# xiejihong0306/collision-detect-GJK-EPA

Hardware: AMD Instinct MI355X
Metric: M convex-pair GJK+EPA queries/sec at 1/2/4/8 MI355X; % HBM roofline (higher is better)
Workload: dtype f64

## Files before the change

### collision-detect-gjk-epa_amd/csrc/gjkepa_kernel.h

```cpp
#pragma once
#include <hip/hip_runtime.h>

#include <cstddef>
#include <cstdint>

#ifndef GJKEPA_G0_G
#define GJKEPA_G0_G 4
#endif
#ifndef GJKEPA_G0_K
#define GJKEPA_G0_K 8
#endif
#ifndef GJKEPA_G0_MINW
#define GJKEPA_G0_MINW 2
#endif
#ifndef GJKEPA_G1_G
#define GJKEPA_G1_G 16
#endif
#ifndef GJKEPA_G1_K
#define GJKEPA_G1_K 8
#endif
#ifndef GJKEPA_G1_MINW
#define GJKEPA_G1_MINW 3
#endif
#ifndef GJKEPA_G2_G
// ... 100 lines not shown
#endif
#ifndef GJKEPA_E5_FCAP
#define GJKEPA_E5_FCAP 416
#endif
#ifndef GJKEPA_E5_MINW
#define GJKEPA_E5_MINW 1
#endif
#ifndef GJKEPA_Q_VCAP
#define GJKEPA_Q_VCAP 40
#endif
#ifndef GJKEPA_Q_FCAP
#define GJKEPA_Q_FCAP 64
#endif
#ifndef GJKEPA_C0_G
#define GJKEPA_C0_G 8
#endif
#ifndef GJKEPA_C0_K
#define GJKEPA_C0_K 4
#endif
#ifndef GJKEPA_C0_MINW
#define GJKEPA_C0_MINW 3
#endif
#ifndef GJKEPA_C1_G
#define GJKEPA_C1_G 64
#endif
#ifndef GJKEPA_C1_K
#define GJKEPA_C1_K 4
#endif
#ifndef GJKEPA_C1_MINW
#define GJKEPA_C1_MINW 3
#endif
#ifndef GJKEPA_EPA_SEED
#define GJKEPA_EPA_SEED 1
#endif
#ifndef GJKEPA_GJK_META
#define GJKEPA_GJK_META 1
#endif
#ifndef GJKEPA_CONTACT_META
#define GJKEPA_CONTACT_META 1
#endif
#ifndef GJKEPA_E1_PRIO
#define GJKEPA_E1_PRIO 2
#endif
#ifndef GJKEPA_HORIZON_W16
#define GJKEPA_HORIZON_W16 1
#endif
#ifndef GJKEPA_SCREEN_SINGLE
#define GJKEPA_SCREEN_SINGLE 1
#endif
#ifndef GJKEPA_EPA_HPACK
#define GJKEPA_EPA_HPACK 1
#endif
#ifndef GJKEPA_PAD_V0
#define GJKEPA_PAD_V0 1
#endif
#ifndef GJKEPA_EMPTY_INF
#define GJKEPA_EMPTY_INF 1
#endif
#ifndef GJKEPA_DOTS_FMAX
#define GJKEPA_DOTS_FMAX 1
#endif
#ifndef GJKEPA_EPA_PLACE
#define GJKEPA_EPA_PLACE 1
#endif
#ifndef GJKEPA_LDS_SKEW
#define GJKEPA_LDS_SKEW 1
// ... 25 lines not shown
#ifndef GJKEPA_E2_LH
#define GJKEPA_E2_LH 0
#endif
#ifndef GJKEPA_E3_LH
#define GJKEPA_E3_LH 1
#endif
#ifndef GJKEPA_E4_LH
#define GJKEPA_E4_LH 1
#endif
#ifndef GJKEPA_E5_LH
#define GJKEPA_E5_LH 0
#endif
#ifndef GJKEPA_C0_LH
#define GJKEPA_C0_LH 1
#endif
#ifndef GJKEPA_C1_LH
#define GJKEPA_C1_LH 1
#endif
#ifndef GJKEPA_CONTACT_OVERLAP
#define GJKEPA_CONTACT_OVERLAP 1
#endif
#define GJKEPA_GJK_TIERS 3
#define GJKEPA_EPA_TIERS 6
#define GJKEPA_CONTACT_TIERS 2

#define GJKEPA_WS_COUNTERS 40
#define GJKEPA_WS_TALLY 48
#define GJKEPA_ROUTE_DONE 0
#define GJKEPA_ROUTE_GJK1 1
#define GJKEPA_ROUTE_EPA0 0x10
#define GJKEPA_ROUTE_CT0 0x20
#define GJKEPA_ROUTE_CT(t) (GJKEPA_ROUTE_CT0 + 2 * (t))
#define GJKEPA_ROUTE_REDO 0x2E

#ifndef GJKEPA_PARK
#define GJKEPA_PARK 1
#endif
#define GJKEPA_PARK_VC 72
#define GJKEPA_PARK_FC 128
#define GJKEPA_PARK_HDR 128
#define GJKEPA_PARK_BYTES (GJKEPA_PARK_HDR + 3 * 8 * GJKEPA_PARK_VC + 2 * 4 * GJKEPA_PARK_FC)

#define GJKEPA_GRID_UNITS (-2)

struct gjkepa_gjk_args {
    const void* verts;
    const int64_t* hull_off;
    const int32_t* hull_cnt;
    const int32_t* pairs;
    int64_t n_pairs;
    uint8_t* route;
    int route_code;
    uint32_t* ctr;
    int claim;
    uint32_t* tally;
    uint32_t* warm;
    void* out;
    int grid;
    int num_cus;
    uint32_t guard;
};

struct gjkepa_epa_args {
    int version;
    double tol_ff;
    const void* verts;
// ... 85 lines not shown
```

### collision-detect-gjk-epa_amd/csrc/gjkepa_kernel.hip

```cpp
#include <hip/hip_runtime.h>

#include <cfloat>
#include <cmath>
#include <cstdint>
#include <type_traits>

#include "../../include/gjkepa.h"
#include "gjkepa_kernel.h"
#include "gk_common.h"

#ifdef GK_PART
#define GK_IN(p) (GK_PART == (p))
#else
#define GK_IN(p) 1
#endif

namespace gk {

constexpr int ST_DEFER = 100;
constexpr int ST_REDO = 103;
constexpr int ST_PARKED = 104;

DEV void gk_lds_fence() { asm volatile("" ::: "memory"); }
#ifndef GJKEPA_SCREEN_FENCE_MIN_G
#define GJKEPA_SCREEN_FENCE_MIN_G 32
#endif
#ifndef GJKEPA_DOTS_FENCE_MIN_G
#define GJKEPA_DOTS_FENCE_MIN_G 64
#endif

template <typename T> DEV constexpr bool certify() { return sizeof(T) == 4; }
template <typename T> DEV bool redo_status(int r, bool last_tier) {
    if constexpr (!certify<T>()) return false;
    return r == ST_REDO || r == GJKEPA_STATUS_EPA_MAXITER || r == GJKEPA_STATUS_DEGENERATE || (r == ST_DEFER && last_tier);
}

[[maybe_unused]] static __constant__ double kDirTab[100][3] = {
#include "dirtab.inc"
};

#ifdef GJKEPA_DIAG_STAMPS
constexpr int kStamps = 32;
__device__ unsigned long long g_stamps[kStamps];
__shared__ unsigned long long s_stamp[kStamps + 1];
DEV void stamp(int id) {
    const uint64_t t = __builtin_amdgcn_s_memtime();
    const uint64_t act = __ballot(1);
    if ((uint64_t)lane_id() == (uint64_t)__builtin_ctzll(act)) { s_stamp[id] += t - s_stamp[kStamps]; s_stamp[kStamps] = t; }
}
DEV void stamp_begin() {
    if (lane_id() == 0) {
        for (int i = 0; i < kStamps; ++i) s_stamp[i] = 0;
        s_stamp[kStamps] = __builtin_amdgcn_s_memtime();
    }
}
DEV void stamp_end() {
    if (lane_id() == 0)
        for (int i = 0; i < kStamps; ++i) if (s_stamp[i]) atomicAdd(&g_stamps[i], s_stamp[i]);
}
#define GK_STAMP(id) stamp(id)
#define GK_STAMP_BEGIN() stamp_begin()
#define GK_STAMP_END() stamp_end()
#elif defined(GJKEPA_DIAG_MARKERS)
#define GK_STAMP(id) asm volatile("; GKMARK %0" ::"n"(id))
#define GK_STAMP_BEGIN() ((void)0)
#define GK_STAMP_END() ((void)0)
#else
// ... 693 lines not shown
        if (f < FC && !(F.fv[r] & kEmpty)) {
            int rk = 0;
            for (int j = 0; j < hw; ++j) rk += E.x.o.key[j] < F.key[r];
            E.x.o.ord[rk] = F.fv[r];
        }
    }
    __builtin_amdgcn_wave_barrier();
    T sx = 0, sy = 0, sz = 0;
    for (int j = 0; j < 3; ++j)
        for (int f = 0; f < nf; ++f) {
            const V3<T> q = c.vert((int)((E.x.o.ord[f] >> (8 * j)) & 0xffu));
            sx += q.x; sy += q.y; sz += q.z;
        }
    __builtin_amdgcn_wave_barrier();
    const T cnt = (T)(nf * 3);
    return vmk<T>(sx / cnt, sy / cnt, sz / cnt);
}

constexpr int ST_CONT = 101;

template <typename T, int R> struct EpaState {
    Faces<T, R> F;
    int nv, hw, nf, F1, iters;
    uint32_t kbase;
    T minv;
    V3<T> dir;
    bool neg;
    int av;
    bool unchanged;
    T hsup;
};
#define EPAST_T EpaState<T, (FC + G - 1) / G>

CTX_T DEV int epa_begin(CTX& c, EPAST_T& S, V3<T> s0, V3<T> s1, V3<T> s2, V3<T> s3) {
    constexpr int R = (FC + G - 1) / G;
    auto& E = c.L.u.e;
    const V3<T> O = zero3<T>();
    const int gl = c.g.gl;
#pragma unroll
    for (int r = 0; r < R; ++r) {
        free_slot(S.F, r);
        const int f = r * G + gl;
        if (f < FC) E.dsv[f] = qnan<T>();
    }
    S.nv = 0; S.hw = 0; S.nf = 0; S.kbase = 0; S.iters = 1; S.F1 = 4; S.unchanged = false;
    const int fq = gl & 3;
    const V3<T> fa = fq == 3 ? s1 : s0, fb = (fq == 0 || fq == 2) ? s1 : s2, fc = fq == 0 ? s2 : s3;
    const V3<T> nq = uninml(fa, fb, fc);
    if (c.g.unib(quad_any(is_zero_nml(nq)))) return GJKEPA_STATUS_DEGENERATE;
    const T dq = fabs(dot(vsub(O, fa), nq));
    const T d0 = qbcast<0>(dq), d1 = qbcast<1>(dq), d2 = qbcast<2>(dq), d3 = qbcast<3>(dq);
    T minv = d0;
    int kmin = 0;
    if (d1 < minv) { minv = d1; kmin = 1; }
    if (d2 < minv) { minv = d2; kmin = 2; }
    if (d3 < minv) { minv = d3; kmin = 3; }
    V3<T> dir = quad_pick(fq == kmin, nq);
    const V3<T> a1 = kmin == 3 ? s1 : s0;
    if (gl < 4) E.dsv[gl] = dq;
    T dt = dot(vsub(a1, O), dir);
    if (c.g.unib(fabs(dt) < Tol<T>::ZO)) {
        const T sx = ((((((((((s0.x + s0.x) + s0.x) + s1.x) + s1.x) + s2.x) + s1.x) + s2.x) + s2.x) + s3.x) + s3.x) + s3.x;
        const T sy = ((((((((((s0.y + s0.y) + s0.y) + s1.y) + s1.y) + s2.y) + s1.y) + s2.y) + s2.y) + s3.y) + s3.y) + s3.y;
        const T sz = ((((((((((s0.z + s0.z) + s0.z) + s1.z) + s1.z) + s2.z) + s1.z) + s2.z) + s2.z) + s3.z) + s3.z) + s3.z;
        const T cnt = (T)12;
        dt = dot(vsub(a1, vmk<T>(sx / cnt, sy / cnt, sz / cnt)), dir);
    }
    if (c.g.unib(dt <= -Tol<T>::ZO)) dir = vneg(dir);
    GK_STAMP(SE_IT1);
    const V3<T> sp = support(c, dir);
    if constexpr (certify<T>()) { S.minv = minv; S.hsup = dot(sp, dir); }
    const bool two = c.g.unib(fabs(minv) < Tol<T>::ZO);
    const bool u1 = !veq(s1, s0);
    const bool u2 = !veq(s2, s0) && !veq(s2, s1);
    const bool u3 = !veq(s3, s0) && !veq(s3, s1) && !veq(s3, s2);
    const int i1 = 1, i2 = u1 ? 2 : 1, i3 = i2 + (u2 ? 1 : 0), isp = i3 + (u3 ? 1 : 0);
    int m = isp + 1;
    V3<T> sq = zero3<T>();
    if (two) { sq = support(c, vneg(dir)); ++m; }
    V3<T> q = s0;
    bool w = gl == 0;
    if (u1 && gl == i1) { q = s1; w = true; }
    if (u2 && gl == i2) { q = s2; w = true; }
    if (u3 && gl == i3) { q = s3; w = true; }
    if (gl == isp) { q = sp; w = true; }
    if (two && gl == isp + 1) { q = sq; w = true; }
    if (w) { E.vx[gl] = q.x; E.vy[gl] = q.y; E.vz[gl] = q.z; }
    __builtin_amdgcn_wave_barrier();
    GK_STAMP(SE_IT1);
    return hull_build(c, S.F, S.kbase, S.hw, S.nv, S.nf, m);
}

constexpr int ST_FALLBACK = 102;
CTX_T DEV int epa_seed(CTX& c, EPAST_T& S, V3<T> s0, V3<T> s1, V3<T> s2, V3<T> s3) {
    constexpr int R = (FC + G - 1) / G;
    auto& E = c.L.u.e;
    const V3<T> O = zero3<T>();
    const int gl = c.g.gl;
    const bool distinct = !veq(s1, s0) && !veq(s2, s0) && !veq(s2, s1) && !veq(s3, s0) && !veq(s3, s1) && !veq(s3, s2);
    if (!c.g.unib(distinct)) return ST_FALLBACK;
    const V3<T> e1 = vsub(s1, s0);
    const T l1 = norm2(e1);
    if (!c.g.unib(l1 > Tol<T>::HULL)) return ST_FALLBACK;
    const V3<T> c2 = cross(e1, vsub(s2, s0));
    if (!c.g.unib(norm2(c2) / l1 > Tol<T>::HULL)) return ST_FALLBACK;
    const V3<T> pn = utzvec(c2);
    if (!c.g.unib(fabs(dot(vsub(s3, s0), pn)) > Tol<T>::HULL)) return ST_FALLBACK;
#pragma unroll
    for (int r = 0; r < R; ++r) {
        free_slot(S.F, r);
        const int f = r * G + gl;
        if (f < FC) E.dsv[f] = qnan<T>();
    }
    S.iters = 1; S.F1 = 4; S.unchanged = false;
    const int fq = gl & 3;
    const V3<T> fa = fq == 3 ? s1 : s0, fb = (fq == 0 || fq == 2) ? s1 : s2, fc = fq == 0 ? s2 : s3;
    const V3<T> nq = uninml(fa, fb, fc);
    if (c.g.unib(quad_any(is_zero_nml(nq)))) return GJKEPA_STATUS_DEGENERATE;
    const T dq = fabs(dot(vsub(O, fa), nq));
    const T d0 = qbcast<0>(dq), d1 = qbcast<1>(dq), d2 = qbcast<2>(dq), d3 = qbcast<3>(dq);
    T minv = d0;
    int kmin = 0;
    if (d1 < minv) { minv = d1; kmin = 1; }
    if (d2 < minv) { minv = d2; kmin = 2; }
    if (d3 < minv) { minv = d3; kmin = 3; }
    V3<T> dir = quad_pick(fq == kmin, nq);
    const V3<T> a1 = kmin == 3 ? s1 : s0;
    if (gl < 4) E.dsv[gl] = dq;
    T dt = dot(vsub(a1, O), dir);
    if (c.g.unib(fabs(dt) < Tol<T>::ZO)) {
        const T sx = ((((((((((s0.x + s0.x) + s0.x) + s1.x) + s1.x) + s2.x) + s1.x) + s2.x) + s2.x) + s3.x) + s3.x) + s3.x;
        const T sy = ((((((((((s0.y + s0.y) + s0.y) + s1.y) + s1.y) + s2.y) + s1.y) + s2.y) + s2.y) + s3.y) + s3.y) + s3.y;
        const T sz = ((((((((((s0.z + s0.z) + s0.z) + s1.z) + s1.z) + s2.z) + s1.z) + s2.z) + s2.z) + s3.z) + s3.z) + s3.z;
        const T cnt = (T)12;
        dt = dot(vsub(a1, vmk<T>(sx / cnt, sy / cnt, sz / cnt)), dir);
    }
    if (c.g.unib(dt <= -Tol<T>::ZO)) dir = vneg(dir);
    S.dir = dir;
    S.minv = minv;
    if (gl < 4) {
        const V3<T> q = gl == 0 ? s0 : gl == 1 ? s1 : gl == 2 ? s2 : s3;
        E.vx[gl] = q.x; E.vy[gl] = q.y; E.vz[gl] = q.z;
    }
    const V3<T> cen = centroid4(s0, s1, s2, s3);
    bool bad = false;
    if (gl < 4) {
        int a = gl == 3 ? 1 : 0, b = (gl == 0 || gl == 2) ? 1 : 2, d = gl == 0 ? 2 : 3;
        const V3<T> Pa = vsel(gl == 3, s1, s0);
        V3<T> Pb = vsel(gl == 0 || gl == 2, s1, s2);
        V3<T> Pd = vsel(gl == 0, s2, s3);
        const V3<T> n0 = cross(vsub(Pb, Pa), vsub(Pd, Pb));
        if (dot(n0, vsub(Pa, cen)) < T(0)) { int t = b; b = d; d = t; const V3<T> q = Pb; Pb = Pd; Pd = q; }
        const V3<T> n = uninml(Pa, Pb, Pd);
        bad = is_zero_nml(n);
        S.F.nx[0] = n.x; S.F.ny[0] = n.y; S.F.nz[0] = n.z;
        S.F.d[0] = dot(vsub(zero3<T>(), Pa), n);
        S.F.fv[0] = (uint32_t)a | ((uint32_t)b << 8) | ((uint32_t)d << 16);
        S.F.key[0] = (uint32_t)gl;
    }
    __builtin_amdgcn_wave_barrier();
    if (c.g.any(bad)) return GJKEPA_STATUS_DEGENERATE;
    S.nv = 4; S.nf = 4; S.kbase = 4; S.hw = 4;
    GK_STAMP(SE_IT1);
    return 0;
}

CTX_T DEV int epa_close(CTX& c, EPAST_T& S, T& depth, V3<T>& normal) {
    const int F2 = S.nf;
    const T prev = S.minv;
    face_argmin(c, S.F, S.minv, S.dir, S.neg, S.av);
    if constexpr (certify<T>()) {
        if (c.g.unib(S.minv < prev - Tol<T>::CERT_DROP * prev)) return ST_REDO;
    }
    V3<T> dir2 = S.dir;
    if (c.g.unib(!S.neg && S.minv > T(0))) dir2 = vneg(dir2);
    bool stop;
    if (S.F1 == F2) stop = S.unchanged || sorted_equal(c, S.F, S.hw);
    else stop = S.F1 > F2;
    GK_STAMP(SE_TERM);
    if constexpr (certify<T>()) {
        if (stop) {
            constexpr int R = (FC + G - 1) / G;
            bool out = false;
#pragma unroll
            for (int r = 0; r < R; ++r) out = out || (!(S.F.fv[r] & kEmpty) && !(S.F.d[r] < T(0)));
            const float sc = c.vmax_a + c.vmax_b;
            const uint32_t bw = c.L.u.e.bestv;
// ... 107 lines not shown
    const T* vx = reinterpret_cast<const T*>(rec + GJKEPA_PARK_HDR);
    const uint32_t* fv = reinterpret_cast<const uint32_t*>(rec + kParkFaces);
    S.nv = c.g.uni((int)hdr[0]); S.hw = c.g.uni((int)hdr[1]); S.nf = c.g.uni((int)hdr[2]); S.F1 = c.g.uni((int)hdr[3]);
    S.iters = c.g.uni((int)hdr[4]); S.kbase = hdr[5]; S.neg = hdr[6] != 0; S.av = (int)hdr[7]; gjk_it = hdr[8];
    S.dir = vmk<T>(tv[0], tv[1], tv[2]);
    S.minv = tv[3];
    S.hsup = tv[4];
    S.unchanged = false;
    for (int i = gl; i < S.nv; i += G) {
        E.vx[i] = vx[i];
        E.vy[i] = vx[GJKEPA_PARK_VC + i];
        E.vz[i] = vx[2 * GJKEPA_PARK_VC + i];
    }
    __builtin_amdgcn_wave_barrier();
#pragma unroll
    for (int r = 0; r < R; ++r) {
        const int f = r * G + gl;
        free_slot(S.F, r);
        if (f < S.hw) {
            const uint32_t w = fv[f];
            if (!(w & kEmpty)) {
                const V3<T> U = c.vert((int)(w & 0xffu)), W = c.vert((int)((w >> 8) & 0xffu)), P = c.vert((int)((w >> 16) & 0xffu));
                const V3<T> n = uninml(U, W, P);
                S.F.nx[r] = n.x; S.F.ny[r] = n.y; S.F.nz[r] = n.z;
                S.F.d[r] = dot(vsub(zero3<T>(), U), n);
                S.F.fv[r] = w;
                S.F.key[r] = fv[GJKEPA_PARK_FC + f];
            }
        }
    }
}

CTX_T DEV int epa(CTX& c, V3<T> s0, V3<T> s1, V3<T> s2, V3<T> s3, T& depth, V3<T>& normal, int& iters, int& nf,
                  bool park = false, ParkCtl pk = {}, const unsigned char* rec = nullptr, uint32_t* gjk_it = nullptr) {
    EPAST_T S;
    int st;
    if (rec) {
        epa_resume(c, S, rec, *gjk_it);
        st = epa_grow(c, S, false);
    } else {
        st = epa_begin(c, S, s0, s1, s2, s3);
        if (st == 0) st = ST_CONT;
    }
    while (st == ST_CONT) {
        st = epa_close(c, S, depth, normal);
        if (st != ST_CONT) break;
        if constexpr (VC <= GJKEPA_PARK_VC && FC <= GJKEPA_PARK_FC) {
            if (park && park_now(c, S, pk)) { st = ST_PARKED; break; }
        }
        st = epa_grow(c, S, false);
    }
    iters = S.iters;
    nf = S.nf;
    return st;
}

CTX_T DEV void scan_top2(CTX& c, int side, V3<T> n, int& i0, int& i1) {
    T mx = -Tol<T>::BIG;
    i0 = -1; i1 = -1;
    const int cnt = side ? c.nb : c.na;
    for (int i = 0; i < cnt; ++i) {
        T t = dot(n, side ? c.B(i) : c.A(i));
        if (t > mx - Tol<T>::PT) { mx = t; i1 = i0; i0 = i; }
    }
    if (i1 == -1) i1 = i0;
}

CTX_T DEV T hull_dot_max(CTX& c, int side, V3<T> n) {
    T mx = -Tol<T>::BIG;
#pragma unroll
    for (int k = 0; k < K; ++k) {
        int i = k * G + c.g.gl;
        const V3<T> p = side ? c.BV(k) : c.AV(k);
        T t = n.x * p.x + n.y * p.y + n.z * p.z;
// ... 440 lines not shown
    k1 = (k == 0 || k == 3) ? c2 : c1;
    k2 = k == 2 ? c2 : c3;
    k3 = km;
}

constexpr double kWarmMargin = 1e-6;
constexpr uint32_t kWarmMiss = 0xFFFFFFFEu;
CTX_T DEV bool warm_start(CTX& c, const uint32_t* w, uint32_t* kc) {
    uint32_t code[4];
    bool ok = true;
#pragma unroll
    for (int i = 0; i < 4; ++i) {
        code[i] = w[i];
        ok = ok && code[i] != kStale && (int)(code[i] & 0xffffu) < c.na && (int)(code[i] >> 16) < c.nb;
    }
    if (!c.g.unib(ok)) return false;
    const V3<T> s0 = decode_pt(c, code[0]), s1 = decode_pt(c, code[1]), s2 = decode_pt(c, code[2]), s3 = decode_pt(c, code[3]);
    const V3<T> M = centroid4(s0, s1, s2, s3), O = zero3<T>();
    const V3<T> P[4] = {s0, s1, s2, s3};
    const int F[4][3] = {{0, 2, 3}, {0, 1, 3}, {0, 1, 2}, {1, 2, 3}};
    bool inside = true;
#pragma unroll
    for (int f = 0; f < 4; ++f) {
        V3<T> n = face_nml(P[F[f][0]], P[F[f][1]], P[F[f][2]]);
        if (dot(n, vsub(P[F[f][0]], M)) < T(0)) n = vneg(n);
        inside = inside && dot(vsub(P[F[f][0]], O), n) > T(kWarmMargin);
    }
    if (!c.g.unib(inside)) return false;
#pragma unroll
    for (int i = 0; i < 4; ++i) kc[i] = code[i];
    return true;
}

CTX_T DEV int gjk_phase(CTX& c, uint32_t* kc, int& gjk_it, bool try_axis = false) {
    const V3<T> O = zero3<T>();
    auto& L = c.L;
    const int gl = c.g.gl;
    gjk_it = 0;
    bool axis_sep = false;
    {
        T cs[(6 + G - 1) / G];
#pragma unroll
        for (int j0 = 0; j0 < 6; j0 += G) {
            const int j = j0 + gl;
            cs[j0 / G] = T(0);
            if (j < 6) {
                const int h = j / 3, ax = j - 3 * (j / 3);
#if GJKEPA_HULL_AOS
                const TH* col = &L.hv[h][0].x + ax;
                constexpr int CS = 4;
#else
                const TH* col = ax == 0 ? L.hx[h] : ax == 1 ? L.hy[h] : L.hz[h];
                constexpr int CS = 1;
#endif
                const int n = h ? c.nb : c.na;
                T sum = 0;
                int i = 0;
                for (; i + 8 <= n; i += 8) {
                    TH v[8];
#pragma unroll
                    for (int u = 0; u < 8; ++u) v[u] = col[CS * (i + u)];
#pragma unroll
                    for (int u = 0; u < 8; ++u) sum += (T)v[u];
                }
                for (; i < n; ++i) sum += (T)col[CS * i];
                cs[j0 / G] = sum / (T)n;
            }
// ... 22 lines not shown
#pragma unroll
            for (int k = 0; k < K; ++k) {
                const int i = k * G + gl;
                const V3<T> pa = c.AV(k), pb = c.BV(k);
                const T ta = d.x * pa.x + d.y * pa.y + d.z * pa.z;
                const T tb = d.x * pb.x + d.y * pb.y + d.z * pb.z;
                if (i < c.na && ta > amax) amax = ta;
                if (i < c.nb && tb < bmin) bmin = tb;
            }
            amax = gmax<G>(amax);
            bmin = gmin<G>(bmin);
            const T margin = sizeof(T) == 8 ? T(kWarmMargin) : T(1e-4);
            axis_sep = c.g.unib(bmin - amax > margin * norm2(d));
        }
    }
    V3<T> s0 = O, s1 = O, s2 = O, s3 = O;
    uint32_t k0 = kStale, k1 = kStale, k2 = kStale, k3 = kStale;
    V3<T> dir;
    for (int iter = 1;; ++iter) {
        if (iter > 99) return PH_MISS;
        dir = vmk<T>((T)kDirTab[iter - 1][0], (T)kDirTab[iter - 1][1], (T)kDirTab[iter - 1][2]);
        s0 = support_pt(c, dir, k0);
        dir = vneg(dir);
        s1 = support_pt(c, dir, k1);
        if (!c.g.unib(allclose8(s0, s1))) break;
    }
    dir = vec_pl(O, s0, s1);
    s2 = support_pt(c, dir, k2);
    if (c.g.unib(allclose8(s2, s0) || allclose8(s2, s1))) return PH_MISS;
    dir = utzvec(cross(vsub(s1, s0), vsub(s2, s1)));
    const T vd = dot(vsub(O, s2), dir);
    bool enter = false;
    if (c.g.unib(fabs(vd) < Tol<T>::PT) && c.g.unib(inside_tri(s0, s1, s2, O))) enter = true;
    const int q = gl & 3;
    V3<T> nq = zero3<T>();
    T mdq = 0;
    if (!enter) {
        if (c.g.unib(vd < T(0))) dir = vneg(dir);
        s3 = support_pt(c, dir, k3);
        const V3<T> n = uninml(s0, s1, s2);
        if (c.g.unib(is_zero_nml(n))) return GJKEPA_STATUS_DEGENERATE;
        if (c.g.unib(fabs(dot(vsub(s3, s0), n)) < Tol<T>::PT)) return PH_MISS;
        nq = quad_normal(q, s0, s1, s2, s3, mdq);
        if (c.g.unib(quad_inside(q, s0, s1, s2, s3, nq))) enter = true;
    }
    GK_STAMP(SG_INIT);
    if (!enter && axis_sep) return PH_MISS;
    if (!enter) {
        constexpr int HS = (12 + G - 1) / G;
        T h1[HS], h2[HS];
#pragma unroll
        for (int t = 0; t < HS; ++t) { h1[t] = 0; h2[t] = 0; }
        const uint64_t lowg = G == 64 ? ~0ull : ((1ull << (G & 63)) - 1ull);
        const int sh = c.g.lane & ~(G - 1);
        for (int it = 1;; ++it) {
            gjk_it = it;
            if (it > 50) return PH_MISS;
#pragma unroll
            for (int t = 0; t < HS; ++t) {
                const int j = t * G + gl;
                h2[t] = h1[t];
                h1[t] = simplex_coord(j < 12 ? j : 0, s0, s1, s2, s3);
            }
            GK_STAMP(SG_CHK);
            update_simplex_c(c, nq, s0, s1, s2, s3, k0, k1, k2, k3);
            nq = quad_normal(q, s0, s1, s2, s3, mdq);
            GK_STAMP(SG_UPD);
            if (c.g.unib(qbcast<2>(mdq) < Tol<T>::PT)) return PH_MISS;
            const V3<T> n = vmk<T>(qbcast<2>(nq.x), qbcast<2>(nq.y), qbcast<2>(nq.z));
            if (c.g.unib(fabs(dot(vsub(s3, s0), n)) < Tol<T>::PT)) return PH_MISS;
            if (c.g.unib(quad_inside(q, s0, s1, s2, s3, nq))) break;
            uint32_t e1 = 0, e2 = 0;
#pragma unroll
            for (int t = 0; t < HS; ++t) {
                const int j = t * G + gl;
                const T cur = simplex_coord(j < 12 ? j : 0, s0, s1, s2, s3);
                e1 |= (uint32_t)((__ballot(fabs(cur - h1[t]) < Tol<T>::PT) >> sh) & lowg) << (t * G);
                e2 |= (uint32_t)((__ballot(fabs(cur - h2[t]) < Tol<T>::PT) >> sh) & lowg) << (t * G);
            }
            e1 &= 0xFFFu;
            e2 &= 0xFFFu;
            bool over = true;
#pragma unroll
            for (int p = 0; p < 4; ++p) over = over && (((e1 >> (3 * p)) & 7u) == 7u || ((e2 >> (3 * p)) & 7u) == 7u);
            if (c.g.unib(over)) return PH_MISS;
        }
        GK_STAMP(SG_CHK);
    }
    kc[0] = k0; kc[1] = k1; kc[2] = k2; kc[3] = k3;
    return PH_HIT;
}

CTX_T DEV int epa_phase(CTX& c, const uint32_t* kc, T& depth, V3<T>& n, uint32_t& diag_epa, bool park = false,
                        ParkCtl pk = {}, const unsigned char* rec = nullptr, uint32_t* gjk_it = nullptr) {
    V3<T> s0 = zero3<T>(), s1 = s0, s2 = s0, s3 = s0;
    if (!rec) { s0 = decode_pt(c, kc[0]); s1 = decode_pt(c, kc[1]); s2 = decode_pt(c, kc[2]); s3 = decode_pt(c, kc[3]); }
    depth = 0;
    n = zero3<T>();
    int eit = 0, nf = 0;
    const int st = epa(c, s0, s1, s2, s3, depth, n, eit, nf, park, pk, rec, gjk_it);
    diag_epa = ((uint32_t)(eit & 0xff) << 8) | ((uint32_t)(nf & 0xffff) << 16);
    return st;
}

CTX_T DEV int contact_phase(CTX& c, T depth, V3<T> n, int version, T tol_ff, T* o13) {
    int st;
    int ia, ib;
    GK_STAMP(SE_TERM);
    DotSet<T, K> D;
    support_dots(c, n, D, ia, ib);
    GK_STAMP(SE_NEAR);
    V3<T> pt = zero3<T>();
    int type = (version == 1 || version == 2) ? collision_type(c, D, tol_ff) : 0;
    if (version == 1) st = contact_v1(c, n, D, pt);
    else if (version == 2) st = contact_v2(c, D, pt);
    else if (version == 3) { V3<T> nw; st = contact_v3(c, n, pt, nw); n = nw; }
    else st = GJKEPA_STATUS_BAD_VERSION;
    GK_STAMP(SE_CONT);
    if (st) return st;
    if (version == 3) type = collision_type(c, n, tol_ff);
    GK_STAMP(SE_TYPE);
    const V3<T> q1 = c.A(ia), q2 = c.B(ib);
    __builtin_amdgcn_wave_barrier();
    o13[0] = depth;
    o13[1] = n.x; o13[2] = n.y; o13[3] = n.z;
    o13[4] = pt.x; o13[5] = pt.y; o13[6] = pt.z;
    o13[7] = q1.x; o13[8] = q1.y; o13[9] = q1.z;
    o13[10] = q2.x; o13[11] = q2.y; o13[12] = q2.z;
    return -type;
}

CTX_T DEV bool load_hulls(CTX& c, const TH* __restrict__ pa, const TH* __restrict__ pb) {
    const int gl = c.g.gl;
// ... 233 lines not shown
    GK_STAMP_BEGIN();
    if (tier_empty(a.tally, a.route_code)) return;
    tally_begin();
    const int claim = pick_claim(a.tally, a.route_code, a.n_pairs, a.claim);
    auto body = [&](int64_t pair, const PairMeta& pm) {
        GK_STAMP(SG_ROUTE);
        Ctx<T, TIn, G, K, 0, 0, LH> c{L, grp};
        const int na = grp.uni(pm.na), nb = grp.uni(pm.nb);
        T o13[13];
#pragma unroll
        for (int i = 0; i < 13; ++i) o13[i] = T(0);
        uint8_t next = 0;
        if (na < 1 || nb < 1 || na > GJKEPA_MAX_HULL_VERTS || nb > GJKEPA_MAX_HULL_VERTS) {
            store_record<G, T>(a.out, pair, gl, o13, 0, 0, GJKEPA_STATUS_BAD_INPUT, 0u);
            if (WARM && gl < 4) a.warm[4 * pair + gl] = kStale;
        } else if (na > K * G || nb > K * G) {
            next = (uint8_t)((na > nb ? na : nb) <= GJKEPA_G1_G * GJKEPA_G1_K ? GJKEPA_ROUTE_GJK1 : GJKEPA_ROUTE_GJK1 + 1);
        } else {
            c.na = na;
            c.nb = nb;
            const bool bad_in = load_hulls(c, verts + pm.oa, verts + pm.ob);
            GK_STAMP(SG_LOAD);
            if (bad_in) {
                store_record<G, T>(a.out, pair, gl, o13, 0, 0, GJKEPA_STATUS_BAD_INPUT, 0u);
                if (WARM && gl < 4) a.warm[4 * pair + gl] = kStale;
            } else {
                uint32_t kc[4];
                int gjk_it = 0;
                int r = PH_MISS;
                bool warm_hit = false;
                if constexpr (WARM) {
                    if (a.warm[4 * pair] != kWarmMiss) warm_hit = warm_start(c, a.warm + 4 * pair, kc);
                }
                if (warm_hit) r = PH_HIT;
                else r = gjk_phase(c, kc, gjk_it, GJKEPA_AXIS_REJECT != 0);
                __builtin_amdgcn_wave_barrier();
                GK_STAMP(SG_CHK);
                if (WARM && gl < 4)
                    a.warm[4 * pair + gl] = r == PH_HIT ? (gl == 0 ? kc[0] : gl == 1 ? kc[1] : gl == 2 ? kc[2] : kc[3])
                                          : (r == PH_MISS && gl == 0) ? kWarmMiss : kStale;
                if (r == PH_HIT) {
#pragma unroll
                    for (int j0 = 0; j0 < 6; j0 += G) {
                        const int j = j0 + gl;
                        const uint32_t word = j == 0 ? kc[0] : j == 1 ? kc[1] : j == 2 ? kc[2] : j == 3 ? kc[3] : j == 4 ? (uint32_t)gjk_it : 0u;
                        if (j < 6) reinterpret_cast<uint32_t*>(a.out)[pair * (sizeof(T) == 8 ? 32 : 16) + j] = word;
                    }
                    next = (uint8_t)(GJKEPA_ROUTE_EPA0 + epa_tier_for(na > nb ? na : nb));
                } else if (r == PH_MISS) {
                    store_record<G, T>(a.out, pair, gl, o13, 0, 0, 0, 0u);
                } else if (certify<T>()) {
                    next = GJKEPA_ROUTE_REDO;
                } else {
                    store_record<G, T>(a.out, pair, gl, o13, 1, 0, r, (uint32_t)(gjk_it & 0xff));
                }
            }
        }
        if (gl == 0) { a.route[pair] = next; tally_route(next); }
        __builtin_amdgcn_wave_barrier();
        GK_STAMP(SG_STORE);
    };
#if GJKEPA_GJK_META
    for_each_routed_pair<G, true>(grp, a.n_pairs, a.route, a.route_code, a.ctr, claim, false, body, a.pairs, a.hull_cnt,
                                  a.hull_off);
#else
    for_each_routed_pair<G>(grp, a.n_pairs, a.route, a.route_code, a.ctr, claim, false, [&](int64_t pair) {
        const int32_t ha = a.pairs[2 * pair], hb = a.pairs[2 * pair + 1];
        body(pair, PairMeta{a.hull_cnt[ha], a.hull_cnt[hb], a.hull_off[ha], a.hull_off[hb]});
    });
#endif
    GK_STAMP(SG_ROUTE);
    tally_end(a.tally);
    GK_STAMP_END();
}

DEV int contact_tier_for(int nmax) { return nmax <= GJKEPA_C0_G * GJKEPA_C0_K ? 0 : 1; }

template <typename TIn, typename T, int G, int K, int VC, int FC, int MINW, bool LH, int PR>
__global__ __launch_bounds__(64, MINW) void epa_kernel(const gjkepa_epa_args a) {
// ... 1 lines not shown
    extern __shared__ __align__(16) unsigned char smem[];
    const Grp<G> grp;
    L_t& L = *reinterpret_cast<L_t*>(smem + lds_stride<L_t, G>() * (grp.lane / G));
    const int gl = grp.gl;
    const TIn* verts = (const TIn*)a.verts;
    GK_GUARD(2, a.route_code);
    GK_STAMP_BEGIN();
    if (tier_empty(a.tally, a.route_code)) return;
    tally_begin();
    const int claim = pick_claim(a.tally, a.route_code, a.n_pairs, a.claim);
    for_each_routed_pair<G>(grp, a.n_pairs, a.route, a.route_code, a.ctr, claim, false, [&](int64_t pair) {
        GK_STAMP(SE_ROUTE);
        Ctx<T, TIn, G, K, VC, FC, LH> c{L, grp};
        const int32_t ha = a.pairs[2 * pair], hb = a.pairs[2 * pair + 1];
        c.na = grp.uni(a.hull_cnt[ha]);
        c.nb = grp.uni(a.hull_cnt[hb]);
        uint32_t* slot = reinterpret_cast<uint32_t*>(a.out) + pair * (sizeof(T) == 8 ? 32 : 16);
        uint32_t kc[4];
        kc[0] = slot[0]; kc[1] = slot[1]; kc[2] = slot[2]; kc[3] = slot[3];
        const uint32_t gjk_it = slot[4];
        load_hulls(c, verts + a.hull_off[ha], verts + a.hull_off[hb]);
        T depth;
        V3<T> n;
        uint32_t de = 0;
        GK_STAMP(SE_LOAD);
#ifdef GJKEPA_DIAG_GJK_ONLY
        const int r = GJKEPA_STATUS_DEGENERATE;
        depth = 0; n = zero3<T>();
#else
        const uint32_t parked = (PR & 2) && a.park ? slot[5] : 0u;
        uint32_t it_park = gjk_it;
        const ParkCtl pk{a.park, a.park_ctr, a.park_cap, gjk_it, slot};
        const bool can_park = (PR & 1) && a.park && a.next_code >= 0;
        const int r = (c.na > G * K || c.nb > G * K) ? ST_DEFER
                    : epa_phase(c, kc, depth, n, de, can_park, pk,
                                parked ? a.park + (size_t)(parked - 1) * GJKEPA_PARK_BYTES : nullptr, &it_park);
#endif
        __builtin_amdgcn_wave_barrier();
        const uint32_t diag = (gjk_it & 0xffu) | de;
        uint8_t next = 0;
        if ((r == ST_DEFER || r == ST_PARKED) && a.next_code >= 0) {
            next = (uint8_t)(GJKEPA_ROUTE_EPA0 + epa_tier_for(c.na > c.nb ? c.na : c.nb, a.next_code - GJKEPA_ROUTE_EPA0, VC));
        } else if (redo_status<T>(r, a.next_code < 0)) {
            next = GJKEPA_ROUTE_REDO;
        } else if (r == 0) {
            T* rec = reinterpret_cast<T*>(slot);
            if (gl < 4) rec[gl] = gl == 0 ? depth : gl == 1 ? n.x : gl == 2 ? n.y : n.z;
            if (gl == 4) slot[sizeof(T) == 8 ? 27 : 14] = diag;
            next = (uint8_t)(a.ct_base + contact_tier_for(c.na > c.nb ? c.na : c.nb));
        } else {
            T o13[13];
#pragma unroll
            for (int i = 0; i < 13; ++i) o13[i] = T(0);
            store_record<G, T>(a.out, pair, gl, o13, 1, 0, r == ST_DEFER ? GJKEPA_STATUS_DEGENERATE : r, diag);
        }
        if (gl == 0) { a.route[pair] = next; tally_route(next); }
        __builtin_amdgcn_wave_barrier();
        GK_STAMP(SE_STORE);
    });
    GK_STAMP(SE_ROUTE);
    tally_end(a.tally);
    GK_STAMP_END();
}

struct PairQueue {
    const uint8_t* route;
    Units U;
    int64_t ch, p0;
    uint32_t* ctr;
// ... 70 lines not shown
            if (gl == 4 % G) slot[sizeof(T) == 8 ? 27 : 14] = diag;
            next = (uint8_t)(a.ct_base + contact_tier_for(c.na > c.nb ? c.na : c.nb));
        } else {
            T o13[13];
#pragma unroll
            for (int i = 0; i < 13; ++i) o13[i] = T(0);
            store_record<G, T>(a.out, pair, gl, o13, 1, 0, r == ST_DEFER ? GJKEPA_STATUS_DEGENERATE : r, diag);
        }
        if (gl == 0) { a.route[pair] = next; tally_route(next); }
    };
    for (;;) {
        const uint64_t idle = __ballot(gl == 0 && !active);
        const int nidle = popc(idle);
        bool fresh = false;
        if (!q.done && (nidle >= REFILL || nidle == NG)) {
#pragma unroll
            for (int g = 0; g < NG; ++g) {
                if ((idle >> (g * G)) & 1ull) {
                    const int64_t p = q.pop();
                    if (p >= 0 && gid == g) { pair = p; fresh = true; }
                }
            }
        }
        if (!__ballot(active || fresh)) break;
        GK_STAMP(SE_ROUTE);
        if (fresh) {
            const int32_t ha = a.pairs[2 * pair], hb = a.pairs[2 * pair + 1];
            c.na = a.hull_cnt[ha];
            c.nb = a.hull_cnt[hb];
            const uint32_t* slot = reinterpret_cast<const uint32_t*>(a.out) + pair * (sizeof(T) == 8 ? 32 : 16);
            uint32_t kc[4];
            kc[0] = slot[0]; kc[1] = slot[1]; kc[2] = slot[2]; kc[3] = slot[3];
            gjk_it = slot[4];
            load_hulls(c, verts + a.hull_off[ha], verts + a.hull_off[hb]);
            S.iters = 1; S.nf = 0;
            int r = ST_DEFER;
            seeded = false;
            if (c.na <= G * K && c.nb <= G * K) {
                const V3<T> s0 = decode_pt(c, kc[0]), s1 = decode_pt(c, kc[1]), s2 = decode_pt(c, kc[2]), s3 = decode_pt(c, kc[3]);
#if GJKEPA_EPA_SEED
                r = epa_seed(c, S, s0, s1, s2, s3);
                seeded = r == 0;
                if (r == ST_FALLBACK)
#endif
                    r = epa_begin(c, S, s0, s1, s2, s3);
            }
            __builtin_amdgcn_wave_barrier();
            active = r == 0;
            if (!active) finish(r, T(0), zero3<T>());
        }
        GK_STAMP(SE_LOAD);
        if (active) {
            T depth = 0;
            V3<T> n = zero3<T>();
            int r = ST_CONT;
            if (!seeded) r = epa_close(c, S, depth, n);
            if constexpr ((PR & 1) != 0) {
                if (r == ST_CONT && !seeded && a.park && a.next_code >= 0) {
                    const ParkCtl pk{a.park, a.park_ctr, a.park_cap, gjk_it,
                                     reinterpret_cast<uint32_t*>(a.out) + pair * (sizeof(T) == 8 ? 32 : 16)};
                    if (park_now(c, S, pk)) r = ST_PARKED;
                }
            }
            if (r == ST_CONT) r = epa_grow(c, S, seeded);
            seeded = false;
            __builtin_amdgcn_wave_barrier();
            if (r != ST_CONT) {
                finish(r, depth, n);
                active = false;
            }
        }
        GK_STAMP(SE_STORE);
    }
    GK_STAMP_END();
    tally_end(a.tally);
}

template <typename TIn, typename T, int K> using QLds = Lds<T, TIn, 64, K, GJKEPA_E5_VCAP, GJKEPA_E5_FCAP, true>;
// ... 459 lines not shown
```

Measured before the change: 180.0.

## Hand off GJK face normals and tetra validity to EPA via output slot

In f64, GJK now stores the four unit face normals of its final tetrahedron and a validity flag in the per-pair output slot. EPA begin and seed stages load them, then skip recomputing the normals and the first-tetrahedron degeneracy checks. This removes redundant cross-product, normalisation and validity work at EPA start. In exchange it adds global stores and loads per pair plus extra route tallies, and it needs the stored normals to be bit-identical with the recomputed ones.

```diff
diff --git a/collision-detect-gjk-epa_amd/csrc/gjkepa_kernel.h b/collision-detect-gjk-epa_amd/csrc/gjkepa_kernel.h
--- a/collision-detect-gjk-epa_amd/csrc/gjkepa_kernel.h
+++ b/collision-detect-gjk-epa_amd/csrc/gjkepa_kernel.h
@@ -156,6 +156,9 @@
 #endif
 #ifndef GJKEPA_EPA_SEED
 #define GJKEPA_EPA_SEED 1
+#endif
+#ifndef GJKEPA_SEED_HANDOFF
+#define GJKEPA_SEED_HANDOFF 1
 #endif
 #ifndef GJKEPA_GJK_META
 #define GJKEPA_GJK_META 1
@@ -247,6 +250,8 @@
 #define GJKEPA_ROUTE_CT0 0x20
 #define GJKEPA_ROUTE_CT(t) (GJKEPA_ROUTE_CT0 + 2 * (t))
 #define GJKEPA_ROUTE_REDO 0x2E
+#define GJKEPA_TALLY_SEED_OWN 0x2D
+#define GJKEPA_TALLY_SEED_HANDED 0x2F
 
 #ifndef GJKEPA_PARK
 #define GJKEPA_PARK 1
diff --git a/collision-detect-gjk-epa_amd/csrc/gjkepa_kernel.hip b/collision-detect-gjk-epa_amd/csrc/gjkepa_kernel.hip
--- a/collision-detect-gjk-epa_amd/csrc/gjkepa_kernel.hip
+++ b/collision-detect-gjk-epa_amd/csrc/gjkepa_kernel.hip
@@ -33,6 +33,38 @@
 template <typename T> DEV bool redo_status(int r, bool last_tier) {
     if constexpr (!certify<T>()) return false;
     return r == ST_REDO || r == GJKEPA_STATUS_EPA_MAXITER || r == GJKEPA_STATUS_DEGENERATE || (r == ST_DEFER && last_tier);
+}
+
+template <typename T> DEV constexpr bool handoff() { return GJKEPA_SEED_HANDOFF != 0 && sizeof(T) == 8; }
+constexpr int kSeedNmlWord = 6, kSeedFlagWord = 30;
+template <typename T> struct SeedOut {
+    V3<T> nq;
+    bool ok;
+};
+template <typename T> struct SeedIn {
+    V3<T> nq;
+    bool on;
+};
+template <typename T> DEV SeedIn<T> no_seed() { return SeedIn<T>{zero3<T>(), false}; }
+template <typename T> DEV SeedIn<T> load_seed(const uint32_t* slot, int gl) {
+    SeedIn<T> h = no_seed<T>();
+    if constexpr (handoff<T>()) {
+        const T* np = reinterpret_cast<const T*>(slot + kSeedNmlWord) + 3 * (gl & 3);
+        h.nq = vmk<T>(np[0], np[1], np[2]);
+        h.on = slot[kSeedFlagWord] == 1u;
+    }
+    return h;
+}
+template <typename T, typename GR> DEV bool simplex_is_first_tetra(const GR& g, V3<T> s0, V3<T> s1, V3<T> s2, V3<T> s3) {
+    const bool distinct = !veq(s1, s0) && !veq(s2, s0) && !veq(s2, s1) && !veq(s3, s0) && !veq(s3, s1) && !veq(s3, s2);
+    if (!g.unib(distinct)) return false;
+    const V3<T> e1 = vsub(s1, s0);
+    const T l1 = norm2(e1);
+    if (!g.unib(l1 > Tol<T>::HULL)) return false;
+    const V3<T> c2 = cross(e1, vsub(s2, s0));
+    if (!g.unib(norm2(c2) / l1 > Tol<T>::HULL)) return false;
+    const V3<T> pn = utzvec(c2);
+    return g.unib(fabs(dot(vsub(s3, s0), pn)) > Tol<T>::HULL);
 }
 
 [[maybe_unused]] static __constant__ double kDirTab[100][3] = {
@@ -792,7 +824,7 @@
 };
 #define EPAST_T EpaState<T, (FC + G - 1) / G>
 
-CTX_T DEV int epa_begin(CTX& c, EPAST_T& S, V3<T> s0, V3<T> s1, V3<T> s2, V3<T> s3) {
+CTX_T DEV int epa_begin(CTX& c, EPAST_T& S, V3<T> s0, V3<T> s1, V3<T> s2, V3<T> s3, SeedIn<T> h = no_seed<T>()) {
     constexpr int R = (FC + G - 1) / G;
     auto& E = c.L.u.e;
     const V3<T> O = zero3<T>();
@@ -806,8 +838,11 @@
     S.nv = 0; S.hw = 0; S.nf = 0; S.kbase = 0; S.iters = 1; S.F1 = 4; S.unchanged = false;
     const int fq = gl & 3;
     const V3<T> fa = fq == 3 ? s1 : s0, fb = (fq == 0 || fq == 2) ? s1 : s2, fc = fq == 0 ? s2 : s3;
-    const V3<T> nq = uninml(fa, fb, fc);
-    if (c.g.unib(quad_any(is_zero_nml(nq)))) return GJKEPA_STATUS_DEGENERATE;
+    V3<T> nq = h.nq;
+    if (!h.on) {
+        nq = uninml(fa, fb, fc);
+        if (c.g.unib(quad_any(is_zero_nml(nq)))) return GJKEPA_STATUS_DEGENERATE;
+    }
     const T dq = fabs(dot(vsub(O, fa), nq));
     const T d0 = qbcast<0>(dq), d1 = qbcast<1>(dq), d2 = qbcast<2>(dq), d3 = qbcast<3>(dq);
     T minv = d0;
@@ -852,20 +887,12 @@
 }
 
 constexpr int ST_FALLBACK = 102;
-CTX_T DEV int epa_seed(CTX& c, EPAST_T& S, V3<T> s0, V3<T> s1, V3<T> s2, V3<T> s3) {
+CTX_T DEV int epa_seed(CTX& c, EPAST_T& S, V3<T> s0, V3<T> s1, V3<T> s2, V3<T> s3, SeedIn<T> h = no_seed<T>()) {
     constexpr int R = (FC + G - 1) / G;
     auto& E = c.L.u.e;
     const V3<T> O = zero3<T>();
     const int gl = c.g.gl;
-    const bool distinct = !veq(s1, s0) && !veq(s2, s0) && !veq(s2, s1) && !veq(s3, s0) && !veq(s3, s1) && !veq(s3, s2);
-    if (!c.g.unib(distinct)) return ST_FALLBACK;
-    const V3<T> e1 = vsub(s1, s0);
-    const T l1 = norm2(e1);
-    if (!c.g.unib(l1 > Tol<T>::HULL)) return ST_FALLBACK;
-    const V3<T> c2 = cross(e1, vsub(s2, s0));
-    if (!c.g.unib(norm2(c2) / l1 > Tol<T>::HULL)) return ST_FALLBACK;
-    const V3<T> pn = utzvec(c2);
-    if (!c.g.unib(fabs(dot(vsub(s3, s0), pn)) > Tol<T>::HULL)) return ST_FALLBACK;
+    if (!h.on && !simplex_is_first_tetra(c.g, s0, s1, s2, s3)) return ST_FALLBACK;
 #pragma unroll
     for (int r = 0; r < R; ++r) {
         free_slot(S.F, r);
@@ -875,8 +902,11 @@
     S.iters = 1; S.F1 = 4; S.unchanged = false;
     const int fq = gl & 3;
     const V3<T> fa = fq == 3 ? s1 : s0, fb = (fq == 0 || fq == 2) ? s1 : s2, fc = fq == 0 ? s2 : s3;
-    const V3<T> nq = uninml(fa, fb, fc);
-    if (c.g.unib(quad_any(is_zero_nml(nq)))) return GJKEPA_STATUS_DEGENERATE;
+    V3<T> nq = h.nq;
+    if (!h.on) {
+        nq = uninml(fa, fb, fc);
+        if (c.g.unib(quad_any(is_zero_nml(nq)))) return GJKEPA_STATUS_DEGENERATE;
+    }
     const T dq = fabs(dot(vsub(O, fa), nq));
     const T d0 = qbcast<0>(dq), d1 = qbcast<1>(dq), d2 = qbcast<2>(dq), d3 = qbcast<3>(dq);
     T minv = d0;
@@ -910,9 +940,13 @@
         V3<T> Pb = vsel(gl == 0 || gl == 2, s1, s2);
         V3<T> Pd = vsel(gl == 0, s2, s3);
         const V3<T> n0 = cross(vsub(Pb, Pa), vsub(Pd, Pb));
-        if (dot(n0, vsub(Pa, cen)) < T(0)) { int t = b; b = d; d = t; const V3<T> q = Pb; Pb = Pd; Pd = q; }
-        const V3<T> n = uninml(Pa, Pb, Pd);
-        bad = is_zero_nml(n);
+        const bool swap = dot(n0, vsub(Pa, cen)) < T(0);
+        if (swap) { int t = b; b = d; d = t; const V3<T> q = Pb; Pb = Pd; Pd = q; }
+        V3<T> n = nq;
+        if (!h.on || swap) {
+            n = uninml(Pa, Pb, Pd);
+            bad = is_zero_nml(n);
+        }
         S.F.nx[0] = n.x; S.F.ny[0] = n.y; S.F.nz[0] = n.z;
         S.F.d[0] = dot(vsub(zero3<T>(), Pa), n);
         S.F.fv[0] = (uint32_t)a | ((uint32_t)b << 8) | ((uint32_t)d << 16);
@@ -1086,14 +1120,15 @@
 }
 
 CTX_T DEV int epa(CTX& c, V3<T> s0, V3<T> s1, V3<T> s2, V3<T> s3, T& depth, V3<T>& normal, int& iters, int& nf,
-                  bool park = false, ParkCtl pk = {}, const unsigned char* rec = nullptr, uint32_t* gjk_it = nullptr) {
+                  bool park = false, ParkCtl pk = {}, const unsigned char* rec = nullptr, uint32_t* gjk_it = nullptr,
+                  SeedIn<T> h = no_seed<T>()) {
     EPAST_T S;
     int st;
     if (rec) {
         epa_resume(c, S, rec, *gjk_it);
         st = epa_grow(c, S, false);
     } else {
-        st = epa_begin(c, S, s0, s1, s2, s3);
+        st = epa_begin(c, S, s0, s1, s2, s3, h);
         if (st == 0) st = ST_CONT;
     }
     while (st == ST_CONT) {
@@ -1600,7 +1635,7 @@
     return true;
 }
 
-CTX_T DEV int gjk_phase(CTX& c, uint32_t* kc, int& gjk_it, bool try_axis = false) {
+CTX_T DEV int gjk_phase(CTX& c, uint32_t* kc, int& gjk_it, bool try_axis = false, SeedOut<T>* so = nullptr) {
     const V3<T> O = zero3<T>();
     auto& L = c.L;
     const int gl = c.g.gl;
@@ -1689,6 +1724,7 @@
     const T vd = dot(vsub(O, s2), dir);
     bool enter = false;
     if (c.g.unib(fabs(vd) < Tol<T>::PT) && c.g.unib(inside_tri(s0, s1, s2, O))) enter = true;
+    const bool tri = enter;
     const int q = gl & 3;
     V3<T> nq = zero3<T>();
     T mdq = 0;
@@ -1745,17 +1781,25 @@
         GK_STAMP(SG_CHK);
     }
     kc[0] = k0; kc[1] = k1; kc[2] = k2; kc[3] = k3;
+    if constexpr (handoff<T>()) {
+        if (so) {
+            const bool same_bits = c.g.unib(quad_all(mdq > T(4) * Tol<T>::Z && nq.x != T(0) && nq.y != T(0) && nq.z != T(0)));
+            so->nq = nq;
+            so->ok = !tri && same_bits && simplex_is_first_tetra(c.g, s0, s1, s2, s3);
+        }
+    }
     return PH_HIT;
 }
 
 CTX_T DEV int epa_phase(CTX& c, const uint32_t* kc, T& depth, V3<T>& n, uint32_t& diag_epa, bool park = false,
-                        ParkCtl pk = {}, const unsigned char* rec = nullptr, uint32_t* gjk_it = nullptr) {
+                        ParkCtl pk = {}, const unsigned char* rec = nullptr, uint32_t* gjk_it = nullptr,
+                        SeedIn<T> h = no_seed<T>()) {
     V3<T> s0 = zero3<T>(), s1 = s0, s2 = s0, s3 = s0;
     if (!rec) { s0 = decode_pt(c, kc[0]); s1 = decode_pt(c, kc[1]); s2 = decode_pt(c, kc[2]); s3 = decode_pt(c, kc[3]); }
     depth = 0;
     n = zero3<T>();
     int eit = 0, nf = 0;
-    const int st = epa(c, s0, s1, s2, s3, depth, n, eit, nf, park, pk, rec, gjk_it);
+    const int st = epa(c, s0, s1, s2, s3, depth, n, eit, nf, park, pk, rec, gjk_it, h);
     diag_epa = ((uint32_t)(eit & 0xff) << 8) | ((uint32_t)(nf & 0xffff) << 16);
     return st;
 }
@@ -2055,8 +2099,9 @@
                 if constexpr (WARM) {
                     if (a.warm[4 * pair] != kWarmMiss) warm_hit = warm_start(c, a.warm + 4 * pair, kc);
                 }
+                SeedOut<T> so{zero3<T>(), false};
                 if (warm_hit) r = PH_HIT;
-                else r = gjk_phase(c, kc, gjk_it, GJKEPA_AXIS_REJECT != 0);
+                else r = gjk_phase(c, kc, gjk_it, GJKEPA_AXIS_REJECT != 0, &so);
                 __builtin_amdgcn_wave_barrier();
                 GK_STAMP(SG_CHK);
                 if (WARM && gl < 4)
@@ -2068,6 +2113,15 @@
                         const int j = j0 + gl;
                         const uint32_t word = j == 0 ? kc[0] : j == 1 ? kc[1] : j == 2 ? kc[2] : j == 3 ? kc[3] : j == 4 ? (uint32_t)gjk_it : 0u;
                         if (j < 6) reinterpret_cast<uint32_t*>(a.out)[pair * (sizeof(T) == 8 ? 32 : 16) + j] = word;
+                    }
+                    if constexpr (handoff<T>()) {
+                        uint32_t* slot = reinterpret_cast<uint32_t*>(a.out) + pair * 32;
+                        if (so.ok && gl < 4) {
+                            const int f = gl == 0 ? 1 : gl == 1 ? 2 : gl == 2 ? 0 : 3;
+                            T* np = reinterpret_cast<T*>(slot + kSeedNmlWord) + 3 * f;
+                            np[0] = so.nq.x; np[1] = so.nq.y; np[2] = so.nq.z;
+                        }
+                        if (gl == 0) slot[kSeedFlagWord] = so.ok ? 1u : 0u;
                     }
                     next = (uint8_t)(GJKEPA_ROUTE_EPA0 + epa_tier_for(na > nb ? na : nb));
                 } else if (r == PH_MISS) {
@@ -2135,9 +2189,12 @@
         uint32_t it_park = gjk_it;
         const ParkCtl pk{a.park, a.park_ctr, a.park_cap, gjk_it, slot};
         const bool can_park = (PR & 1) && a.park && a.next_code >= 0;
-        const int r = (c.na > G * K || c.nb > G * K) ? ST_DEFER
+        const bool fits = c.na <= G * K && c.nb <= G * K;
+        const SeedIn<T> seed = load_seed<T>(slot, gl);
+        if (fits && !parked && gl == 0) tally_route(seed.on ? GJKEPA_TALLY_SEED_HANDED : GJKEPA_TALLY_SEED_OWN);
+        const int r = !fits ? ST_DEFER
                     : epa_phase(c, kc, depth, n, de, can_park, pk,
-                                parked ? a.park + (size_t)(parked - 1) * GJKEPA_PARK_BYTES : nullptr, &it_park);
+                                parked ? a.park + (size_t)(parked - 1) * GJKEPA_PARK_BYTES : nullptr, &it_park, seed);
 #endif
         __builtin_amdgcn_wave_barrier();
         const uint32_t diag = (gjk_it & 0xffu) | de;
@@ -2274,18 +2331,20 @@
             uint32_t kc[4];
             kc[0] = slot[0]; kc[1] = slot[1]; kc[2] = slot[2]; kc[3] = slot[3];
             gjk_it = slot[4];
+            const SeedIn<T> seed = load_seed<T>(slot, gl);
             load_hulls(c, verts + a.hull_off[ha], verts + a.hull_off[hb]);
             S.iters = 1; S.nf = 0;
             int r = ST_DEFER;
             seeded = false;
             if (c.na <= G * K && c.nb <= G * K) {
                 const V3<T> s0 = decode_pt(c, kc[0]), s1 = decode_pt(c, kc[1]), s2 = decode_pt(c, kc[2]), s3 = decode_pt(c, kc[3]);
+                if (gl == 0) tally_route(seed.on ? GJKEPA_TALLY_SEED_HANDED : GJKEPA_TALLY_SEED_OWN);
 #if GJKEPA_EPA_SEED
-                r = epa_seed(c, S, s0, s1, s2, s3);
+                r = epa_seed(c, S, s0, s1, s2, s3, seed);
                 seeded = r == 0;
                 if (r == ST_FALLBACK)
 #endif
-                    r = epa_begin(c, S, s0, s1, s2, s3);
+                    r = epa_begin(c, S, s0, s1, s2, s3, seed);
             }
             __builtin_amdgcn_wave_barrier();
             active = r == 0;
```

Measured after the change: 184.4, median of 6. 1.02x the previous value.
